# AntoineBlanot/LC2IS

Measured on AMD Instinct MI355X. Metric: training-step images/sec (512x512, ADE20K-150), higher is better.
Workload: dtype bf16; 1 GPU; BaseModelWithText ViT-B/16 + CLIP-text + decoder + fused head/CE train step, 512x512, 151 classes, text len 16, sgd; batch_per_gpu=32, global_batch=32, parallelism=dp1

## Files before the change

include/lc2is_hip.h:

```cpp
#ifndef LC2IS_HIP_H
#define LC2IS_HIP_H
#include <stddef.h>
#include <stdint.h>

#ifdef __cplusplus
extern "C" {
#endif

#define LC2IS_ACT_NONE 0
#define LC2IS_ACT_QUICK_GELU 1
#define LC2IS_ACT_RELU 2
#define LC2IS_ACT_DQUICK_GELU 3
#define LC2IS_ACT_DRELU 4
#define LC2IS_ACT_QUICK_GELU_GRAD 5
#define LC2IS_ACT_MUL_AUX 6
#define LC2IS_ACT_GELU_ERF 7
#define LC2IS_ACT_DGELU_ERF 8
#define LC2IS_ACT_ADD_AUX 9

#define LC2IS_INTERP_BICUBIC 0
#define LC2IS_INTERP_BILINEAR 1

typedef void* lc2is_stream_t;

// ... 103 lines not shown
int lc2is_transpose_bf16_batched(const void* src, int ld_src, long stride_src, void* dst, int ld_dst, long stride_dst,
                                 int R, int C, int batch, lc2is_stream_t stream);

int lc2is_patchify(const float* pixels, void* out_bf16, int ld_out, int B, int H, int W, int patch,
                   lc2is_stream_t stream);
int lc2is_vit_embed_fwd(const float* patch, int ld_patch, const float* cls, const float* pos, float* x,
                        int ldx, int B, int P, int C, lc2is_stream_t stream);
int lc2is_vit_embed_bwd(const float* dx, int ldx, float* dpos, float* dcls, void* dpatch_bf16, int ld_dpatch,
                        int B, int P, int C, int accumulate, lc2is_stream_t stream);
int lc2is_text_embed_fwd(const int64_t* ids, const float* tok, const float* pos, float* x, int ldx, int B,
                         int L, int C, int vocab, lc2is_stream_t stream);
int lc2is_text_embed_bwd(const int64_t* ids, const float* dx, int ldx, float* dtok, float* dpos, int B, int L,
                         int C, int vocab, int accumulate, lc2is_stream_t stream);
int lc2is_rows_copy_f32(const float* src, int S_src, int src_off, float* dst_f32, void* dst_bf16, int S_dst,
                        int dst_off, int B, int n, int C, lc2is_stream_t stream);
int lc2is_rows_copy_bf16(const void* src, int S_src, int src_off, float* dst_f32, void* dst_bf16, int S_dst,
                         int dst_off, int B, int n, int C, lc2is_stream_t stream);

int lc2is_sgd_step(float* params, const float* grads, float* momentum_buf, size_t n, float lr, float momentum,
                   float weight_decay, float grad_scale, lc2is_stream_t stream);
int lc2is_adamw_step(float* params, const float* grads, float* exp_avg, float* exp_avg_sq, size_t n, float lr,
                     float beta1, float beta2, float eps, float weight_decay, int step, float grad_scale,
                     lc2is_stream_t stream);

size_t lc2is_head_upsample_ce_workspace_bytes(int B, int h, int w, int C, int S, int mode, int want_grad);
int lc2is_head_upsample_ce(const float* scores_lo, int ld, const int64_t* labels, float* dscores_lo,
                           float* scores_hi, float* loss_sum, int B, int h, int w, int C, int S, int mode,
                           long ignore_index, float grad_scale, void* workspace, size_t workspace_bytes,
                           lc2is_stream_t stream);
int lc2is_head_upsample_ce_opts(const float* scores_lo, int ld, const int64_t* labels, float* dscores_lo,
                                float* scores_hi, float* loss_sum, int B, int h, int w, int C, int S, int mode,
                                long ignore_index, float grad_scale, const float* class_weight, float label_smoothing,
                                void* workspace, size_t workspace_bytes, lc2is_stream_t stream);
int lc2is_upsample_bwd_nchw(const float* dhi, float* dlo, int ld, int B, int h, int w, int C, int S, int mode,
                            lc2is_stream_t stream);
int lc2is_ce_nchw_fwd(const float* logits, const int64_t* labels, float* lse, float* loss_sum, int B, int C,
                      long HW, long ignore_index, lc2is_stream_t stream);
int lc2is_ce_nchw_bwd(const float* logits, const int64_t* labels, const float* lse, const float* grad_scale_dev,
                      float grad_scale, float* dlogits, int B, int C, long HW, long ignore_index,
                      lc2is_stream_t stream);
int lc2is_ce_nchw_fwd_opts(const float* logits, const int64_t* labels, float* lse, float* loss_sum, float* loss_px,
                           int B, int C, long HW, long ignore_index, const float* class_weight, float label_smoothing,
                           lc2is_stream_t stream);
int lc2is_ce_nchw_bwd_opts(const float* logits, const int64_t* labels, const float* lse, const float* grad_scale_dev,
                           float grad_scale, const float* grad_px, float* dlogits, int B, int C, long HW,
                           long ignore_index, const float* class_weight, float label_smoothing,
// ... 199 lines not shown
```

lc2is_amd/csrc/misc.hip:

```cpp
#include "common.h"
#include "lc2is_hip.h"

namespace {

__global__ __launch_bounds__(256) void shadow_refresh_kernel(const lc2is_shadow_desc* __restrict__ descs,
                                                              int ndesc) {
  __shared__ bf16_t tile[64][66];
  int lo = 0, hi = ndesc - 1;
  const int bid = blockIdx.x;
  while (lo < hi) {
    const int mid = (lo + hi + 1) >> 1;
    if (descs[mid].tile_start <= bid) lo = mid; else hi = mid - 1;
  }
  const lc2is_shadow_desc d = descs[lo];
  const int t = bid - d.tile_start;
  const int tk = (d.K + 63) / 64;
  const int n0 = (t / tk) * 64, k0 = (t % tk) * 64;
  const float* src = (const float*)d.src;
  bf16_t* dst = (bf16_t*)d.dst;
  bf16_t* dstT = (bf16_t*)d.dstT;
  const int tx = threadIdx.x & 15, ty = threadIdx.x >> 4;
#pragma unroll
  for (int r = 0; r < 4; ++r) {
    const int n = n0 + ty + 16 * r, k = k0 + 4 * tx;
// ... 220 lines not shown
    if (dst_b) *reinterpret_cast<uint2*>(dst_b + o) = make_uint2(pack_bf16x2(v.x, v.y), pack_bf16x2(v.z, v.w));
  }
}

__global__ __launch_bounds__(256) void sgd_kernel(float* p, const float* __restrict__ g, float* mom, size_t n4,
                                                   float lr, float momentum, float wd, float gscale) {
  for (size_t i = (size_t)blockIdx.x * 256 + threadIdx.x; i < n4; i += (size_t)gridDim.x * 256) {
    float4 pv = reinterpret_cast<float4*>(p)[i];
    const float4 gv = reinterpret_cast<const float4*>(g)[i];
    float d[4] = {gv.x * gscale + wd * pv.x, gv.y * gscale + wd * pv.y, gv.z * gscale + wd * pv.z,
                  gv.w * gscale + wd * pv.w};
    if (mom) {
      float4 mv = reinterpret_cast<float4*>(mom)[i];
      mv.x = momentum * mv.x + d[0]; mv.y = momentum * mv.y + d[1];
      mv.z = momentum * mv.z + d[2]; mv.w = momentum * mv.w + d[3];
      reinterpret_cast<float4*>(mom)[i] = mv;
      d[0] = mv.x; d[1] = mv.y; d[2] = mv.z; d[3] = mv.w;
    }
    pv.x -= lr * d[0]; pv.y -= lr * d[1]; pv.z -= lr * d[2]; pv.w -= lr * d[3];
    reinterpret_cast<float4*>(p)[i] = pv;
  }
}

__global__ __launch_bounds__(256) void adamw_kernel(float* p, const float* __restrict__ g, float* m, float* v,
                                                     size_t n4, float lr, float b1, float b2, float eps,
                                                     float wd, float bc1, float bc2, float gscale) {
  for (size_t i = (size_t)blockIdx.x * 256 + threadIdx.x; i < n4; i += (size_t)gridDim.x * 256) {
    float4 pv = reinterpret_cast<float4*>(p)[i];
    const float4 gv = reinterpret_cast<const float4*>(g)[i];
    float4 mv = reinterpret_cast<float4*>(m)[i], vv = reinterpret_cast<float4*>(v)[i];
    float* pp = &pv.x; const float* gp = &gv.x; float* mp = &mv.x; float* vp = &vv.x;
#pragma unroll
    for (int k = 0; k < 4; ++k) {
      const float gg = gp[k] * gscale;
      pp[k] *= (1.f - lr * wd);
      mp[k] = b1 * mp[k] + (1.f - b1) * gg;
      vp[k] = b2 * vp[k] + (1.f - b2) * gg * gg;
      const float denom = sqrtf(vp[k]) / sqrtf(bc2) + eps;
      pp[k] -= (lr / bc1) * (mp[k] / denom);
    }
    reinterpret_cast<float4*>(p)[i] = pv;
    reinterpret_cast<float4*>(m)[i] = mv;
    reinterpret_cast<float4*>(v)[i] = vv;
  }
}

// ... 124 lines not shown

extern "C" int lc2is_rows_copy_bf16(const void* src, int S_src, int src_off, float* dst_f32, void* dst_bf16,
                                    int S_dst, int dst_off, int B, int n, int C, lc2is_stream_t stream_) {
  hipStream_t stream = (hipStream_t)stream_;
  if (!src || (!dst_f32 && !dst_bf16)) return LC2IS_ERR_NULL;
  if (B <= 0 || n <= 0 || C <= 0 || C % 4 || src_off < 0 || dst_off < 0 || src_off + n > S_src ||
      dst_off + n > S_dst)
    return LC2IS_ERR_SHAPE;
  hipLaunchKernelGGL(rows_copy_bf16_kernel, dim3(ew_grid((size_t)B * n * C / 4)), dim3(256), 0, stream, (const bf16_t*)src,
                     S_src, src_off, dst_f32, (bf16_t*)dst_bf16, S_dst, dst_off, B, n, C);
  return lc2is_check_launch();
}

extern "C" int lc2is_sgd_step(float* params, const float* grads, float* momentum_buf, size_t n, float lr,
                              float momentum, float weight_decay, float grad_scale, lc2is_stream_t stream_) {
  hipStream_t stream = (hipStream_t)stream_;
  if (!params || !grads) return LC2IS_ERR_NULL;
  if (n == 0 || n % 4) return LC2IS_ERR_SHAPE;
  hipLaunchKernelGGL(sgd_kernel, dim3(ew_grid(n / 4)), dim3(256), 0, stream, params, grads, momentum_buf, n / 4,
                     lr, momentum, weight_decay, grad_scale);
  return lc2is_check_launch();
}

extern "C" int lc2is_adamw_step(float* params, const float* grads, float* exp_avg, float* exp_avg_sq, size_t n,
                                float lr, float beta1, float beta2, float eps, float weight_decay, int step,
                                float grad_scale, lc2is_stream_t stream_) {
  hipStream_t stream = (hipStream_t)stream_;
  if (!params || !grads || !exp_avg || !exp_avg_sq) return LC2IS_ERR_NULL;
  if (n == 0 || n % 4 || step < 1) return LC2IS_ERR_SHAPE;
  const float bc1 = 1.f - powf(beta1, (float)step), bc2 = 1.f - powf(beta2, (float)step);
  hipLaunchKernelGGL(adamw_kernel, dim3(ew_grid(n / 4)), dim3(256), 0, stream, params, grads, exp_avg,
                     exp_avg_sq, n / 4, lr, beta1, beta2, eps, weight_decay, bc1, bc2, grad_scale);
  return lc2is_check_launch();
}
```

lc2is_amd/nn/base.py:

```python
from __future__ import annotations

import torch
from torch import nn

from .. import ops


import os as _os

_WGRAD_SIDE = _os.environ.get("LC2IS_WGRAD_STREAM", "0") == "1"
_wgrad_streams: dict = {}


def wgrad_stream(device) -> torch.cuda.Stream:
    s = _wgrad_streams.get(device)
    if s is None:
        s = _wgrad_streams[device] = torch.cuda.Stream(device)
    return s


class _on_wgrad_stream:

    def __init__(self, *tensors):
        self.tensors = [t for t in tensors if t is not None]
# ... 86 lines not shown

def drop_branch_grad16(ds: DropSites | None, site: str, g32: torch.Tensor, g16: torch.Tensor | None) -> torch.Tensor:
    if ds is None:
        return g16 if g16 is not None else ops.cast_bf16(g32)
    return ops.dropout_rows_f32(g32, ds.p, ds.seeds[site], out_f32=None, out_bf16=True)[1]


def require_cuda(t: torch.Tensor, what: str) -> None:
    if not t.is_cuda:
        raise RuntimeError(
            f"lc2is_amd: {what} is on {t.device}; the MI355X path has no CPU fallback — move the module and its "
            "inputs to a HIP device (the CPU oracle lives in oracle/ and is test-only)")


class HipModule(nn.Module):

    def __init__(self) -> None:
        super().__init__()
        self._sh = None
        self._sh_table = None
        self._sh_versions = None
        self._sh_device = None
        self._sh_ptrs = []
        self._grad_ready_cb = None
        self._part_ready_cb = None

    def _build_shadows(self, device):
        raise NotImplementedError

    def _params_for_version(self):
        return list(self.parameters(recurse=True))

    def _ensure_ready(self):
        ps = self._params_for_version()
        dev = ps[0].device
        require_cuda(ps[0], f"{type(self).__name__} parameters")
        if self._sh is None or self._sh_device != dev or any(p.data_ptr() != q for p, q in zip(ps, self._sh_ptrs)):
            ns, entries = self._build_shadows(dev)
            self._sh = ns
            self._sh_table = ops.ShadowTable(entries, dev) if entries else None
            self._sh_device = dev
            self._sh_ptrs = [p.data_ptr() for p in ps]
            self._sh_versions = None
        vers = [p._version for p in ps]
        if vers != self._sh_versions:
            if self._sh_table is not None:
                self._sh_table.refresh()
            self._post_refresh()
            self._sh_versions = vers
        return self._sh

    def _post_refresh(self):
        pass

    def _grads_ready(self):
        if self._sh_device is not None:
            join_wgrad_stream(self._sh_device)
        if self._grad_ready_cb is not None:
            self._grad_ready_cb(self)

    def _part_grads_ready(self, part: nn.Module):
        if self._part_ready_cb is not None:
            if self._sh_device is not None:
                join_wgrad_stream(self._sh_device)
            self._part_ready_cb(self, part)

    def invalidate_shadows(self):
        self._sh_versions = None

    def _apply(self, fn, *args, **kwargs):
        self._sh = None
        return super()._apply(fn, *args, **kwargs)


def grad_buf(p: torch.Tensor):
    if p.grad is None:
        g = getattr(p, "_lc2is_grad", None)
        if g is None or g.shape != p.shape or g.device != p.device:
            g = torch.empty_like(p)
        p.grad = g
        return g, False
    return p.grad, True


class WgradBatch:

    _active = None

    def __init__(self, enabled: bool = True):
        self.enabled = enabled and _os.environ.get("LC2IS_WGRAD_GROUPED", "1") != "0"
        self.items = []
# ... 53 lines not shown
    return grad_buf(p)


GROUP_SKIP = 255


def granule_group_map(offsets, sizes, group_ids, dead=(), align: int = 64, ngroups: int | None = None) -> torch.Tensor:
    if not (len(offsets) == len(sizes) == len(group_ids)) or not len(offsets):
        raise ValueError("granule_group_map: offsets, sizes and group_ids must be non-empty and of one length")
    top = GROUP_SKIP if ngroups is None else int(ngroups)
    if not 1 <= top <= GROUP_SKIP:
        raise ValueError(f"granule_group_map: ngroups must be 1..{GROUP_SKIP}, got {ngroups}")
    dead = set(dead)
    ids, counts, at = [], [], 0
    for k, (o, n, g) in enumerate(zip(offsets, sizes, group_ids)):
        if o != at or o % align or n < 1:
            raise ValueError(f"granule_group_map: parameter {k} at offset {o} (size {n}) does not continue an aligned layout at {at}")
        if not 0 <= int(g) < top:
            raise ValueError(f"granule_group_map: parameter {k} has group id {g}; ids are 0..{top - 1}")
        ids.append(GROUP_SKIP if k in dead else int(g))
        counts.append((n + align - 1) // align)
        at = o + counts[-1] * align
    return torch.repeat_interleave(torch.tensor(ids, dtype=torch.uint8), torch.tensor(counts, dtype=torch.int64))


class ParamArena:

    ALIGN = 64

    def __init__(self, module: nn.Module):
        params = []
        seen = set()
        for p in module.parameters():
            if id(p) not in seen:
                seen.add(id(p))
                params.append(p)
        if not params:
            raise RuntimeError("ParamArena: module has no parameters")
        dev = params[0].device
        require_cuda(params[0], "ParamArena parameters")
        offs, total = [], 0
        for p in params:
            offs.append(total)
            total += (p.numel() + self.ALIGN - 1) // self.ALIGN * self.ALIGN
        self.flat = torch.zeros(total, dtype=torch.float32, device=dev)
        self.grad = torch.zeros(total, dtype=torch.float32, device=dev)
# ... 71 lines not shown
```

lc2is_amd/ops.py:

```python
from __future__ import annotations

import ctypes as C
import math
import os

import torch

from . import _lib

ACT_NONE, ACT_QUICK_GELU, ACT_RELU, ACT_DQUICK_GELU, ACT_DRELU, ACT_QUICK_GELU_GRAD, ACT_MUL_AUX = 0, 1, 2, 3, 4, 5, 6
ACT_GELU_ERF, ACT_DGELU_ERF, ACT_ADD_AUX = 7, 8, 9

_P, _I, _F, _Z, _L, _U64 = C.c_void_p, C.c_int, C.c_float, C.c_size_t, C.c_long, C.c_ulonglong
_ARGTYPES = {
    "lc2is_gemm_nt_bf16": [_P, _I, _P, _I, _P, _P, _I, _P, _I, _P, _I, _P, _I, _P, _I, _I, _I, _I, _I, _I, _P],
    "lc2is_gemm_nt_ln_xchg_bytes": [_I, _I],
    "lc2is_gemm_nt_ln_bf16": [_P, _I, _P, _I, _P, _P, _I, _P, _I, _P, _P, _F, _P, _I, _P, _P, _P, _Z, _I, _I, _I, _P],
    "lc2is_gemm_nt_bf16_batched": [_P, _I, _L, _P, _I, _L, _P, _I, _L, _P, _I, _L, _I, _I, _I, _I, _P],
    "lc2is_transpose_bf16_batched": [_P, _I, _L, _P, _I, _L, _I, _I, _I, _P],
    "lc2is_gemm_tn_workspace_bytes": [_I, _I, _I],
    "lc2is_gemm_tn_bf16": [_P, _I, _P, _I, _P, _I, _P, _I, _I, _I, _I, _P, _Z, _P],
    "lc2is_colsum_workspace_bytes": [_I, _I],
    "lc2is_colsum_bf16": [_P, _I, _P, _I, _I, _I, _P, _Z, _P],
    "lc2is_layernorm_fwd": [_P, _I, _I, _P, _P, _P, _I, _P, _I, _P, _P, _I, _I, _F, _P],
# ... 5 lines not shown
    "lc2is_attention_fwd": [_P, _I, _P, _I, _P, _I, _P, _I, _P, _P, _I, _I, _I, _I, _I, _F, _I, _P],
    "lc2is_attention_bwd": [_P, _I, _P, _I, _P, _I, _P, _I, _P, _I, _P, _I, _P, _I, _P, _I, _P, _P, _P,
                            _I, _I, _I, _I, _I, _F, _I, _P],
    "lc2is_attention_fwd_dropout": [_P, _I, _P, _I, _P, _I, _P, _I, _P, _P, _I, _I, _I, _I, _I, _F, _I, _F, _U64, _P],
    "lc2is_attention_bwd_dropout": [_P, _I, _P, _I, _P, _I, _P, _I, _P, _I, _P, _I, _P, _I, _P, _I, _P, _P, _P,
                                    _I, _I, _I, _I, _I, _F, _I, _F, _U64, _P],
    "lc2is_dropout_rows_f32": [_P, _I, _P, _I, _P, _I, _P, _I, _I, _I, _I, _F, _U64, _P],
    "lc2is_dropout_rows_bf16": [_P, _I, _P, _I, _I, _I, _F, _U64, _P],
    "lc2is_dropout_mask": [_P, _L, _I, _F, _U64, _P],
    "lc2is_shadow_refresh": [_P, _I, _I, _P],
    "lc2is_set_cu_budget": [_I],
    "lc2is_get_cu_budget": [],
    "lc2is_cast_f32_bf16": [_P, _I, _P, _I, _I, _I, _P],
    "lc2is_transpose_bf16": [_P, _I, _P, _I, _I, _I, _P],
    "lc2is_patchify": [_P, _P, _I, _I, _I, _I, _I, _P],
    "lc2is_vit_embed_fwd": [_P, _I, _P, _P, _P, _I, _I, _I, _I, _P],
    "lc2is_vit_embed_bwd": [_P, _I, _P, _P, _P, _I, _I, _I, _I, _I, _P],
    "lc2is_text_embed_fwd": [_P, _P, _P, _P, _I, _I, _I, _I, _I, _P],
    "lc2is_text_embed_bwd": [_P, _P, _I, _P, _P, _I, _I, _I, _I, _I, _P],
    "lc2is_rows_copy_bf16": [_P, _I, _I, _P, _P, _I, _I, _I, _I, _I, _P],
    "lc2is_rows_copy_f32": [_P, _I, _I, _P, _P, _I, _I, _I, _I, _I, _P],
    "lc2is_sgd_step": [_P, _P, _P, _Z, _F, _F, _F, _F, _P],
    "lc2is_adamw_step": [_P, _P, _P, _P, _Z, _F, _F, _F, _F, _F, _I, _F, _P],
    "lc2is_grad_sumsq_blocks": [_Z],
    "lc2is_grad_sumsq_workspace_bytes": [_Z],
    "lc2is_grad_sumsq": [_P, _Z, _P, _Z, _P],
    "lc2is_optim_ctrl_update": [_P, _P, _P, _I, _P, _I, _F, _F, _I, _F, _F, _P],
    "lc2is_sgd_step_ctrl": [_P, _P, _P, _Z, _P, _F, _F, _I, _P],
    "lc2is_adamw_step_ctrl": [_P, _P, _P, _P, _Z, _P, _F, _F, _F, _F, _I, _P],
    "lc2is_sgd_step_groups": [_P, _P, _P, _Z, _P, _P, _P, _I, _F, _I, _P],
    "lc2is_adamw_step_groups": [_P, _P, _P, _P, _Z, _P, _P, _P, _I, _F, _F, _F, _I, _P],
    "lc2is_ema_update_ctrl": [_P, _P, _Z, _P, _F, _I, _I, _I, _P],
    "lc2is_swap_f32": [_P, _P, _Z, _P],
    "lc2is_head_upsample_ce_workspace_bytes": [_I, _I, _I, _I, _I, _I, _I],
    "lc2is_head_upsample_ce": [_P, _I, _P, _P, _P, _P, _I, _I, _I, _I, _I, _I, C.c_long, _F, _P, _Z, _P],
    "lc2is_ce_nchw_fwd": [_P, _P, _P, _P, _I, _I, C.c_long, C.c_long, _P],
    "lc2is_ce_nchw_bwd": [_P, _P, _P, _P, _F, _P, _I, _I, C.c_long, C.c_long, _P],
    "lc2is_head_upsample_ce_opts": [_P, _I, _P, _P, _P, _P, _I, _I, _I, _I, _I, _I, C.c_long, _F, _P, _F, _P, _Z, _P],
    "lc2is_ce_nchw_fwd_opts": [_P, _P, _P, _P, _P, _I, _I, C.c_long, C.c_long, _P, _F, _P],
    "lc2is_ce_nchw_fwd_workspace_bytes": [_I, C.c_long],
    "lc2is_ce_nchw_fwd_ordered": [_P, _P, _P, _P, _P, _I, _I, C.c_long, C.c_long, _P, _F, _P, _Z, _P],
    "lc2is_ce_nchw_bwd_opts": [_P, _P, _P, _P, _F, _P, _P, _I, _I, C.c_long, C.c_long, _P, _F, _P],
    "lc2is_upsample_bwd_nchw": [_P, _P, _I, _I, _I, _I, _I, _I, _I, _P],
    "lc2is_head_upsample_px": [_P, _I, _P, _P, _I, _I, _I, _I, _I, _I, _L, _P],
    "lc2is_ohem_select_workspace_bytes": [_L],
    "lc2is_ohem_select": [_P, _P, _P, _L, _I, _L, _F, _L, _P, _P, _Z, _P],
# ... 470 lines not shown
        self._keep = []
        for i, (src, dst, dstT) in enumerate(entries):
            if src.dim() == 1:
                src = src.unsqueeze(0)
                dst = dst.unsqueeze(0) if dst is not None and dst.dim() == 1 else dst
            f32copy = dst is not None and dst.dtype == torch.float32
            _chk(src, torch.float32, "shadow src")
            _chk(dst, torch.float32 if f32copy else torch.bfloat16, "shadow dst")
            _chk(dstT, torch.bfloat16, "shadow dstT")
            if f32copy and dstT is not None:
                raise RuntimeError("lc2is_amd: fp32 shadow copies have no transposed twin")
            if not src.is_contiguous():
                raise RuntimeError("lc2is_amd: shadow source must be contiguous")
            N, K = src.shape
            if K % 4 or (dstT is not None and N % 4):
                raise RuntimeError(f"lc2is_amd: shadow shape [{N},{K}] not supported")
            if dst is not None and tuple(dst.shape) != (N, K):
                raise RuntimeError("lc2is_amd: shadow dst shape mismatch")
            if dstT is not None and tuple(dstT.shape) != (K, N):
                raise RuntimeError("lc2is_amd: shadow dstT shape mismatch")
            descs[i] = ShadowDesc(src.data_ptr(), _ptr(dst), _ptr(dstT), N, K, _ld(dst), _ld(dstT), start, int(f32copy))
            start += ((N + 63) // 64) * ((K + 63) // 64)
            self._keep.append((src, dst, dstT))
        self.n = len(entries)
        self.total_tiles = start
        raw = bytes(descs)
        self.dev = torch.frombuffer(bytearray(raw), dtype=torch.uint8).to(device)

    def refresh(self):
        rc = _fn("lc2is_shadow_refresh")(self.dev.data_ptr(), self.n, self.total_tiles, _stream())
        _lib.check(rc, "shadow_refresh")


def cast_bf16(src: torch.Tensor, out: torch.Tensor | None = None):
    _chk(src, torch.float32, "src")
    M, Cc = src.shape
    out = out if out is not None else torch.empty((M, Cc), dtype=torch.bfloat16, device=src.device)
    _chk(out, torch.bfloat16, "out")
    _lib.check(_fn("lc2is_cast_f32_bf16")(_ptr(src), _ld(src), _ptr(out), _ld(out), M, Cc, _stream()), "cast")
    return out


def transpose_bf16(src: torch.Tensor, out: torch.Tensor | None = None):
    _chk(src, torch.bfloat16, "src")
    R, Cc = src.shape
    out = out if out is not None else torch.empty((Cc, R), dtype=torch.bfloat16, device=src.device)
    _chk(out, torch.bfloat16, "out")
    _lib.check(_fn("lc2is_transpose_bf16")(_ptr(src), _ld(src), _ptr(out), _ld(out), R, Cc, _stream()),
               "transpose")
    return out
# ... 48 lines not shown
    V, Cc = dtok.shape
    _lib.check(_fn("lc2is_text_embed_bwd")(_ptr(ids), _ptr(dx), _ld(dx), _ptr(dtok), _ptr(dpos), B, L, Cc, V,
                                           int(accumulate), _stream()), "text_embed_bwd")


def rows_copy(src, S_src: int, src_off: int, S_dst: int, dst_off: int, B: int, n: int, *, dst_f32=None,
              dst_bf16=None):
    sb = src.dtype == torch.bfloat16
    _chk(src, torch.bfloat16 if sb else torch.float32, "src")
    Cc = src.shape[1]
    if not src.is_contiguous() or src.shape[0] != B * S_src:
        raise RuntimeError("lc2is_amd.rows_copy: src must be contiguous [B*S_src, C]")
    for t in (dst_f32, dst_bf16):
        if t is not None and (not t.is_contiguous() or tuple(t.shape) != (B * S_dst, Cc)):
            raise RuntimeError("lc2is_amd.rows_copy: dst must be contiguous [B*S_dst, C]")
    _lib.check(_fn("lc2is_rows_copy_bf16" if sb else "lc2is_rows_copy_f32")(_ptr(src), S_src, src_off, _ptr(dst_f32), _ptr(dst_bf16),
                                                                            S_dst, dst_off, B, n, Cc, _stream()), "rows_copy")


def sgd_step(params, grads, momentum_buf, lr, momentum=0.0, weight_decay=0.0, grad_scale=1.0):
    _chk(params, torch.float32, "params", 1); _chk(grads, torch.float32, "grads", 1)
    _lib.check(_fn("lc2is_sgd_step")(_ptr(params), _ptr(grads), _ptr(momentum_buf), params.numel(), lr, momentum,
                                     weight_decay, grad_scale, _stream()), "sgd_step")


def adamw_step(params, grads, m, v, lr, beta1, beta2, eps, weight_decay, step, grad_scale=1.0):
    _chk(params, torch.float32, "params", 1); _chk(grads, torch.float32, "grads", 1)
    _lib.check(_fn("lc2is_adamw_step")(_ptr(params), _ptr(grads), _ptr(m), _ptr(v), params.numel(), lr, beta1,
                                       beta2, eps, weight_decay, int(step), grad_scale, _stream()), "adamw_step")


OPTIM_CTRL_WORDS = 12
(CTRL_CALLS, CTRL_APPLIED, CTRL_SKIPPED, CTRL_FINITE, CTRL_GRAD_NORM, CTRL_CLIP_COEF, CTRL_LR, CTRL_BC1, CTRL_BC2, CTRL_GRAD_MUL,
 CTRL_APPLY) = range(11)


def _chk_ctrl(ctrl):
    _chk(ctrl, torch.int32, "ctrl", 1)
    if ctrl.numel() != OPTIM_CTRL_WORDS:
        raise RuntimeError(f"lc2is_amd: ctrl must be an int32 [{OPTIM_CTRL_WORDS}] control block (lc2is_optim_ctrl)")


def _chk_same_numel(name, params, *others):
    for t in others:
        if t is not None:
            _chk(t, torch.float32, name + " buffer", 1)
# ... 920 lines not shown
```

lc2is_amd/step.py:

```python
from __future__ import annotations

import contextlib
import math
import os
import re

import torch
from torch import nn

from . import ops
from .nn.base import HipModule, ParamArena


_DEFAULT_LR = 1e-5


def _accepts_ohem(model) -> bool:
    import inspect
    fl = getattr(model, "forward_loss", None)
    return fl is not None and "ohem" in inspect.signature(fl).parameters


def _accepts_dice(model) -> bool:
    import inspect
    fl = getattr(model, "forward_loss", None)
    return fl is not None and "dice" in inspect.signature(fl).parameters


def lr_table_from_torch(make_scheduler, base_lr: float, steps: int) -> torch.Tensor:
    if steps < 1:
        raise ValueError("lr_table_from_torch: steps must be >= 1")
    opt = torch.optim.SGD([torch.nn.Parameter(torch.zeros(1))], lr=base_lr)
    sched = make_scheduler(opt)
    rates = []
# ... 188 lines not shown
            depth[m.group(1)] = max(depth.get(m.group(1), 0), int(m.group(2)) + 1)
    merged = {}
    for name, prm in named:
        wd = float(weight_decay)
        if no_decay and (prm.dim() == 1 or name.endswith(("position_embedding.weight", "token_embedding.weight"))
                         or any(sub in name for sub in extra)):
            wd = 0.0
        scale, best = 1.0, -1
        for prefix, f in lr_scales.items():
            if name.startswith(prefix) and len(prefix) > best:
                scale, best = float(f), len(prefix)
        if layer_decay is not None:
            m = _TOWER_LAYER.match(name)
            if m:
                scale *= float(layer_decay) ** (depth[m.group(1)] - int(m.group(2)))
            else:
                for tower, L in depth.items():
                    if name.startswith((tower + ".embeddings.", tower + ".pre_layrnorm.")):
                        scale *= float(layer_decay) ** (L + 1)
        merged.setdefault((scale, wd), []).append(name)
    return [dict(params=names, lr_scale=scale, weight_decay=wd) for (scale, wd), names in merged.items()]


class TrainStep:

    def __init__(self, model: nn.Module, *, optimizer: str = "sgd", lr: float = _DEFAULT_LR, momentum: float = 0.0,
                 weight_decay: float = 0.0, betas=(0.9, 0.999), eps: float = 1e-8, reducer=None,
                 ignore_index: int | None = None, criterion: nn.Module | None = None, lr_schedule=None,
                 schedule_steps: int | None = None, max_grad_norm: float | None = None, skip_nonfinite: bool = False,
                 device_state: bool = False, param_groups=None, ema_decay: float | None = None, ema_warmup: bool = False,
                 ema_every: int = 1) -> None:
        _check_ema_args(ema_decay, ema_warmup, ema_every)
        device_path = bool(device_state or skip_nonfinite or lr_schedule is not None or max_grad_norm is not None
                           or param_groups is not None or ema_decay is not None)
        groups = None
        if param_groups is not None:
            groups, group_of = _resolve_param_groups(model, param_groups, weight_decay)
        if max_grad_norm is not None and not float(max_grad_norm) > 0.0:
            raise ValueError(f"TrainStep: max_grad_norm must be > 0 (or None / inf for no clipping), got {max_grad_norm}")
        table = _lr_table(lr_schedule, schedule_steps, lr) if (device_path or schedule_steps is not None) else None
        self._loss_opts = False
        self._ohem = False
        self._dice = False
        if criterion is not None:
            from .nn.loss import AuxiliaryLoss, CrossEntropyLoss, DiceCrossEntropyLoss, OhemCrossEntropyLoss
            if not isinstance(criterion, (CrossEntropyLoss, nn.CrossEntropyLoss)) or isinstance(criterion, AuxiliaryLoss):
# ... 8 lines not shown
            self._ohem = isinstance(criterion, OhemCrossEntropyLoss)
            if self._ohem and not _accepts_ohem(model):
                raise TypeError("TrainStep: an OhemCrossEntropyLoss needs a model whose forward_loss takes ohem= "
                                "(BaseModelWithText); the compose models do not select hard pixels")
            self._dice = isinstance(criterion, DiceCrossEntropyLoss)
            if self._dice and not _accepts_dice(model):
                raise TypeError("TrainStep: a DiceCrossEntropyLoss needs a model whose forward_loss takes dice= "
                                "(BaseModelWithText); the compose models have no Dice head")
        self.criterion = criterion
        self.model = model
        self.arena = ParamArena(model)
        self.kind = optimizer.lower()
        if self.kind not in ("sgd", "adamw"):
            raise ValueError("TrainStep: optimizer must be 'sgd' or 'adamw'")
        self.lr, self.momentum, self.weight_decay, self.betas, self.eps = lr, momentum, weight_decay, betas, eps
        dev = self.arena.flat.device
        self.mom = torch.zeros_like(self.arena.flat) if (self.kind == "sgd" and momentum != 0.0) else None
        if self.kind == "adamw":
            self.m, self.v = torch.zeros_like(self.arena.flat), torch.zeros_like(self.arena.flat)
        self.t = 0
        self.reducer = reducer
        self.ignore_index = -100 if ignore_index is None else ignore_index
        self._hip_modules = [m for m in model.modules() if isinstance(m, HipModule)]
        if reducer is not None:
            reducer.attach(model, self.arena)
        self._dev = dev
        self._ctrl = None
        if device_path:
            self._ctrl = torch.zeros(ops.OPTIM_CTRL_WORDS, dtype=torch.int32, device=dev)
            self._ctrl_f = self._ctrl.view(torch.float32)
            self.lr_table = table.to(dev)
            self.max_grad_norm = float("inf") if max_grad_norm is None else float(max_grad_norm)
            self.skip_nonfinite = bool(skip_nonfinite)
            self.reverse_walk = False
        self._groups = groups
        if groups is not None:
            self.arena.set_groups([group_of[id(p)] for p in self.arena.params], len(groups))
            self._group_table = torch.tensor([[g["lr_scale"], g["weight_decay"]] for g in groups], dtype=torch.float32).to(dev)
        self.ema, self._ema_swapped = None, False
        self.ema_decay = None if ema_decay is None else float(ema_decay)
        self.ema_warmup, self.ema_every = bool(ema_warmup), int(ema_every)
        if ema_decay is not None:
            self._ema_w = 1.0 - self.ema_decay
            self.ema_reverse_walk = True
            self.ema = self.arena.flat.clone()

# ... 122 lines not shown
        sd = {"format": 1, "meta": self._state_meta(), "t": int(self.t)}
        for k, b in self._state_buffers().items():
            sd[k] = b.detach().to("cpu", copy=True)
        if self._ctrl is not None:
            sd["lr_table"] = self.lr_table.detach().to("cpu", copy=True)
        if self._groups is not None:
            sd["group_table"] = self._group_table.detach().to("cpu", copy=True)
        return sd

    def load_state_dict(self, sd: dict) -> None:
        if self._ema_swapped:
            raise RuntimeError("TrainStep.load_state_dict: not inside ema_weights()")
        if not isinstance(sd, dict) or "meta" not in sd or "t" not in sd:
            raise ValueError("TrainStep.load_state_dict: not a TrainStep.state_dict()")
        check_train_state(sd["meta"], self._state_meta())
        bufs = self._state_buffers()
        for k, b in bufs.items():
            src = sd.get(k)
            if not isinstance(src, torch.Tensor) or src.dtype != b.dtype or src.shape != b.shape:
                raise ValueError(f"TrainStep.load_state_dict: '{k}' must be a {b.dtype} tensor of shape {tuple(b.shape)}")
        for k, b in bufs.items():
            b.copy_(sd[k])
        self.t = int(sd["t"])

    def step(self, inputs: dict, labels: torch.Tensor) -> torch.Tensor:
        if self._ema_swapped:
            raise RuntimeError("TrainStep.step: inside ema_weights() the parameters are the EMA; leave the block before training")
        arena = self.arena
        arena.zero_grad(set_to_none=True)
        if self.reducer is not None:
            self.reducer.begin_step()
        if self._ohem:
            c = self.criterion
            loss = self.model.forward_loss(inputs, labels, self.ignore_index, weight=c.weight,
                                           label_smoothing=float(c.label_smoothing), reduction=c.reduction,
                                           ohem=c.ohem if c.training else None)
            if c.training:
                c.last_labels, c.last_info = self.model.last_ohem
        elif self._dice:
            c = self.criterion
            loss = self.model.forward_loss(inputs, labels, self.ignore_index, dice=c.dice)
            c.last_stats = self.model.last_dice
        elif self._loss_opts:
            c = self.criterion
            loss = self.model.forward_loss(inputs, labels, self.ignore_index, weight=c.weight,
                                           label_smoothing=float(c.label_smoothing), reduction=c.reduction)
        else:
            loss = self.model.forward_loss(inputs, labels, self.ignore_index)
        loss.backward()
        live = arena.finalize_grads()
        gscale = 1.0
        if self.reducer is not None:
            self.reducer.finish_step()
            gscale = 1.0 / self.reducer.world_size
        self.t += 1
        segs = [(0, arena.numel)] if (self.weight_decay == 0.0 or live == [(0, arena.numel)]) else live
        if self._ctrl is not None:
            ctrl = self._ctrl
            b1, b2 = self.betas if self.kind == "adamw" else (0.0, 0.0)
            partials, flags = ops.grad_sumsq(arena.grad)
            ops.optim_ctrl_update(ctrl, partials, flags, self.lr_table, grad_scale=gscale, max_norm=self.max_grad_norm,
                                  skip_nonfinite=self.skip_nonfinite, beta1=b1, beta2=b2)
            if self._groups is not None:
                gmap = arena.group_map()
                if self.kind == "sgd":
                    ops.sgd_step_groups(arena.flat, arena.grad, self.mom, ctrl, gmap, self._group_table, self.momentum,
                                        reverse=self.reverse_walk)
                else:
                    ops.adamw_step_groups(arena.flat, arena.grad, self.m, self.v, ctrl, gmap, self._group_table, self.betas[0],
                                          self.betas[1], self.eps, reverse=self.reverse_walk)
                segs = []
            for lo, hi in segs:
                sl = slice(lo, hi)
                if self.kind == "sgd":
                    ops.sgd_step_ctrl(arena.flat[sl], arena.grad[sl], None if self.mom is None else self.mom[sl], ctrl,
                                      self.momentum, self.weight_decay, reverse=self.reverse_walk)
                else:
                    ops.adamw_step_ctrl(arena.flat[sl], arena.grad[sl], self.m[sl], self.v[sl], ctrl, self.betas[0],
                                        self.betas[1], self.eps, self.weight_decay, reverse=self.reverse_walk)
# ... 19 lines not shown
        if self._ema_swapped:
            raise RuntimeError("TrainStep.capture: inside ema_weights() the parameters are the EMA; leave the block before training")
        if self.kind == "adamw" and self._ctrl is None:
            raise RuntimeError("TrainStep.capture: AdamW bias correction is step-dependent; capture supports SGD")
        if hasattr(self.model, "overlap_text") and os.environ.get("LC2IS_GRAPH_OVERLAP", "1") == "0":
            self.model.overlap_text = False
        from .nn.base import DropoutRng
        DropoutRng.last.clear()
        static_in = {k: v.clone() for k, v in inputs.items()}
        static_lb = labels.clone()
        side = torch.cuda.Stream()
        side.wait_stream(torch.cuda.current_stream())
        with torch.cuda.stream(side):
            for _ in range(warmup):
                self.step(static_in, static_lb)
        torch.cuda.current_stream().wait_stream(side)
        torch.cuda.synchronize()
        if DropoutRng.last:
            raise RuntimeError("TrainStep.capture: the model has active dropout / drop-path sites "
                               f"({len(DropoutRng.last)}); their per-step seeds cannot be captured — train eagerly or set the rates to 0")
        prev = getattr(self, "_captured", None)
        if prev is not None:
            prev.release()
        graph = torch.cuda.CUDAGraph()
        t_before = self.t
        mark0 = ops.captured_tables_mark()
        with torch.cuda.graph(graph, stream=side):
            static_loss = self.step(static_in, static_lb)
        mark1 = ops.captured_tables_mark()
        self.t = t_before

        def replay(new_inputs: dict, new_labels: torch.Tensor) -> torch.Tensor:
            if self._ema_swapped:
                raise RuntimeError("TrainStep replay: inside ema_weights() the parameters are the EMA; leave the block before "
                                   "training")
            for k, v in new_inputs.items():
                if v is not static_in[k]:
                    static_in[k].copy_(v, non_blocking=True)
            if new_labels is not static_lb:
                static_lb.copy_(new_labels, non_blocking=True)
            graph.replay()
            self.t += 1
            return static_loss

        state = {"live": True}

        def release() -> None:
            if not state["live"]:
                return
            state["live"] = False
            torch.cuda.synchronize()
            graph.reset()
            ops.release_captured_tables_range(mark0, mark1)
            if getattr(self, "_captured", None) is replay:
                self._captured = None

        replay.static_inputs, replay.static_labels, replay.graph, replay.release = static_in, static_lb, graph, release
        self._captured = replay
        return replay
```

Before: 1031 images/s.

## Fuse SGD update with bf16 shadow weight refresh in one kernel

Adds an SGD kernel that walks the shadow-table tiles, updates fp32 params and momentum in place, and writes the bf16 (and transposed) shadow copies in the same pass. A segment kernel updates the remaining parameters that have no shadows. Modules are then marked as having current shadows, so the separate refresh pass on the next forward is skipped. This removes one full read of the weights and several launches per step, at the cost of extra version-guard bookkeeping and a new path that only applies to eager SGD without groups, EMA or graph capture.

```diff
diff --git a/include/lc2is_hip.h b/include/lc2is_hip.h
--- a/include/lc2is_hip.h
+++ b/include/lc2is_hip.h
@@ -149,6 +149,14 @@
 int lc2is_adamw_step(float* params, const float* grads, float* exp_avg, float* exp_avg_sq, size_t n, float lr,
                      float beta1, float beta2, float eps, float weight_decay, int step, float grad_scale,
                      lc2is_stream_t stream);
+
+#define LC2IS_MAX_SGD_SEGMENTS 64
+int lc2is_sgd_step_shadow(const lc2is_shadow_desc* descs, int ndesc, int total_tiles, float* params, const float* grads,
+                          float* momentum_buf, size_t n, float lr, float momentum, float weight_decay, float grad_scale,
+                          lc2is_stream_t stream);
+int lc2is_sgd_step_segments(float* params, const float* grads, float* momentum_buf, size_t n, const size_t* seg_lo,
+                            const size_t* seg_hi, int nseg, float lr, float momentum, float weight_decay, float grad_scale,
+                            lc2is_stream_t stream);
 
 size_t lc2is_head_upsample_ce_workspace_bytes(int B, int h, int w, int C, int S, int mode, int want_grad);
 int lc2is_head_upsample_ce(const float* scores_lo, int ld, const int64_t* labels, float* dscores_lo,
diff --git a/lc2is_amd/csrc/misc.hip b/lc2is_amd/csrc/misc.hip
--- a/lc2is_amd/csrc/misc.hip
+++ b/lc2is_amd/csrc/misc.hip
@@ -266,6 +266,105 @@
   }
 }
 
+__device__ __forceinline__ void sgd_update4(float4& pv, const float4 gv, float4& mv, const bool has_mom, const float lr,
+                                            const float momentum, const float wd, const float gscale) {
+  float d[4] = {gv.x * gscale + wd * pv.x, gv.y * gscale + wd * pv.y, gv.z * gscale + wd * pv.z,
+                gv.w * gscale + wd * pv.w};
+  if (has_mom) {
+    mv.x = momentum * mv.x + d[0]; mv.y = momentum * mv.y + d[1];
+    mv.z = momentum * mv.z + d[2]; mv.w = momentum * mv.w + d[3];
+    d[0] = mv.x; d[1] = mv.y; d[2] = mv.z; d[3] = mv.w;
+  }
+  pv.x -= lr * d[0]; pv.y -= lr * d[1]; pv.z -= lr * d[2]; pv.w -= lr * d[3];
+}
+
+__global__ __launch_bounds__(256) void sgd_shadow_kernel(const lc2is_shadow_desc* __restrict__ descs, int ndesc,
+                                                          const float* arena_lo, const float* arena_hi, ptrdiff_t goff,
+                                                          ptrdiff_t moff, int has_mom, float lr, float momentum, float wd,
+                                                          float gscale) {
+  __shared__ bf16_t tile[64][66];
+  int lo = 0, hi = ndesc - 1;
+  const int bid = blockIdx.x;
+  while (lo < hi) {
+    const int mid = (lo + hi + 1) >> 1;
+    if (descs[mid].tile_start <= bid) lo = mid; else hi = mid - 1;
+  }
+  const lc2is_shadow_desc d = descs[lo];
+  const int t = bid - d.tile_start;
+  const int tk = (d.K + 63) / 64;
+  const int n0 = (t / tk) * 64, k0 = (t % tk) * 64;
+  float* src = (float*)d.src;
+  if (src < arena_lo || src + (size_t)d.N * d.K > arena_hi) return;
+  bf16_t* dst = (bf16_t*)d.dst;
+  bf16_t* dstT = (bf16_t*)d.dstT;
+  const int tx = threadIdx.x & 15, ty = threadIdx.x >> 4;
+#pragma unroll
+  for (int r = 0; r < 4; ++r) {
+    const int n = n0 + ty + 16 * r, k = k0 + 4 * tx;
+    float4 v = make_float4(0.f, 0.f, 0.f, 0.f);
+    if (n < d.N && k < d.K) {
+      float* pp = src + (size_t)n * d.K + k;
+      v = *reinterpret_cast<const float4*>(pp);
+      const float4 gv = *reinterpret_cast<const float4*>(pp + goff);
+      float4 mv = make_float4(0.f, 0.f, 0.f, 0.f);
+      if (has_mom) mv = *reinterpret_cast<const float4*>(pp + moff);
+      sgd_update4(v, gv, mv, has_mom != 0, lr, momentum, wd, gscale);
+      if (has_mom) *reinterpret_cast<float4*>(pp + moff) = mv;
+      *reinterpret_cast<float4*>(pp) = v;
+    }
+    const bf16_t b0 = f32_to_bf16(v.x), b1 = f32_to_bf16(v.y), b2 = f32_to_bf16(v.z), b3 = f32_to_bf16(v.w);
+    if (d.flags & 1) {
+      if (dst && n < d.N && k < d.K) *reinterpret_cast<float4*>((float*)d.dst + (size_t)n * d.ld_dst + k) = v;
+    } else if (dst && n < d.N && k < d.K) {
+      uint2 pk = make_uint2((unsigned)b0 | ((unsigned)b1 << 16), (unsigned)b2 | ((unsigned)b3 << 16));
+      *reinterpret_cast<uint2*>(dst + (size_t)n * d.ld_dst + k) = pk;
+    }
+    tile[ty + 16 * r][4 * tx + 0] = b0;
+    tile[ty + 16 * r][4 * tx + 1] = b1;
+    tile[ty + 16 * r][4 * tx + 2] = b2;
+    tile[ty + 16 * r][4 * tx + 3] = b3;
+  }
+  if (!dstT) return;
+  __syncthreads();
+#pragma unroll
+  for (int r = 0; r < 4; ++r) {
+    const int k = k0 + ty + 16 * r, n = n0 + 4 * tx;
+    if (k < d.K && n < d.N) {
+      const int kk = ty + 16 * r;
+      uint2 pk = make_uint2((unsigned)tile[4 * tx][kk] | ((unsigned)tile[4 * tx + 1][kk] << 16),
+                            (unsigned)tile[4 * tx + 2][kk] | ((unsigned)tile[4 * tx + 3][kk] << 16));
+      *reinterpret_cast<uint2*>(dstT + (size_t)k * d.ld_dstT + n) = pk;
+    }
+  }
+}
+
+struct sgd_segs {
+  unsigned lo4[LC2IS_MAX_SGD_SEGMENTS];
+  unsigned pre4[LC2IS_MAX_SGD_SEGMENTS + 1];
+};
+
+__global__ __launch_bounds__(256) void sgd_segments_kernel(float* p, const float* __restrict__ g, float* mom,
+                                                            const sgd_segs segs, int nseg, float lr, float momentum, float wd,
+                                                            float gscale) {
+  __shared__ unsigned s_lo[LC2IS_MAX_SGD_SEGMENTS], s_pre[LC2IS_MAX_SGD_SEGMENTS + 1];
+  if ((int)threadIdx.x < nseg) s_lo[threadIdx.x] = segs.lo4[threadIdx.x];
+  if ((int)threadIdx.x <= nseg) s_pre[threadIdx.x] = segs.pre4[threadIdx.x];
+  __syncthreads();
+  const size_t total = s_pre[nseg];
+  int s = 0;
+  for (size_t j = (size_t)blockIdx.x * 256 + threadIdx.x; j < total; j += (size_t)gridDim.x * 256) {
+    while (j >= s_pre[s + 1]) ++s;
+    const size_t i = (size_t)s_lo[s] + (j - s_pre[s]);
+    float4 pv = reinterpret_cast<float4*>(p)[i];
+    const float4 gv = reinterpret_cast<const float4*>(g)[i];
+    float4 mv = make_float4(0.f, 0.f, 0.f, 0.f);
+    if (mom) mv = reinterpret_cast<float4*>(mom)[i];
+    sgd_update4(pv, gv, mv, mom != nullptr, lr, momentum, wd, gscale);
+    if (mom) reinterpret_cast<float4*>(mom)[i] = mv;
+    reinterpret_cast<float4*>(p)[i] = pv;
+  }
+}
+
 __global__ __launch_bounds__(256) void adamw_kernel(float* p, const float* __restrict__ g, float* m, float* v,
                                                      size_t n4, float lr, float b1, float b2, float eps,
                                                      float wd, float bc1, float bc2, float gscale) {
@@ -436,6 +535,45 @@
   return lc2is_check_launch();
 }
 
+extern "C" int lc2is_sgd_step_shadow(const lc2is_shadow_desc* descs_dev, int ndesc, int total_tiles, float* params,
+                                     const float* grads, float* momentum_buf, size_t n, float lr, float momentum,
+                                     float weight_decay, float grad_scale, lc2is_stream_t stream_) {
+  hipStream_t stream = (hipStream_t)stream_;
+  if (!descs_dev || !params || !grads) return LC2IS_ERR_NULL;
+  if (ndesc <= 0 || total_tiles <= 0 || n == 0 || n % 4 || ((uintptr_t)params & 15u) || ((uintptr_t)grads & 15u) ||
+      ((uintptr_t)momentum_buf & 15u))
+    return LC2IS_ERR_SHAPE;
+  const ptrdiff_t goff = grads - params, moff = momentum_buf ? momentum_buf - params : 0;
+  hipLaunchKernelGGL(sgd_shadow_kernel, dim3(total_tiles), dim3(256), 0, stream, descs_dev, ndesc, (const float*)params,
+                     (const float*)(params + n), goff, moff, momentum_buf ? 1 : 0, lr, momentum, weight_decay, grad_scale);
+  return lc2is_check_launch();
+}
+
+extern "C" int lc2is_sgd_step_segments(float* params, const float* grads, float* momentum_buf, size_t n,
+                                       const size_t* seg_lo, const size_t* seg_hi, int nseg, float lr, float momentum,
+                                       float weight_decay, float grad_scale, lc2is_stream_t stream_) {
+  hipStream_t stream = (hipStream_t)stream_;
+  if (!params || !grads || (nseg > 0 && (!seg_lo || !seg_hi))) return LC2IS_ERR_NULL;
+  if (nseg < 0 || nseg > LC2IS_MAX_SGD_SEGMENTS || n == 0 || n % 4 || (n >> 34) || ((uintptr_t)params & 15u) ||
+      ((uintptr_t)grads & 15u) || ((uintptr_t)momentum_buf & 15u))
+    return LC2IS_ERR_SHAPE;
+  sgd_segs segs = {};
+  size_t total4 = 0, prev_hi = 0;
+  for (int s = 0; s < nseg; ++s) {
+    const size_t lo = seg_lo[s], hi = seg_hi[s];
+    if (lo >= hi || hi > n || lo % 64 || hi % 64 || lo < prev_hi) return LC2IS_ERR_SHAPE;
+    segs.lo4[s] = (unsigned)(lo / 4);
+    segs.pre4[s] = (unsigned)total4;
+    total4 += (hi - lo) / 4;
+    prev_hi = hi;
+  }
+  segs.pre4[nseg] = (unsigned)total4;
+  if (nseg == 0) return 0;
+  hipLaunchKernelGGL(sgd_segments_kernel, dim3(ew_grid(total4)), dim3(256), 0, stream, params, grads, momentum_buf, segs,
+                     nseg, lr, momentum, weight_decay, grad_scale);
+  return lc2is_check_launch();
+}
+
 extern "C" int lc2is_adamw_step(float* params, const float* grads, float* exp_avg, float* exp_avg_sq, size_t n,
                                 float lr, float beta1, float beta2, float eps, float weight_decay, int step,
                                 float grad_scale, lc2is_stream_t stream_) {
diff --git a/lc2is_amd/nn/base.py b/lc2is_amd/nn/base.py
--- a/lc2is_amd/nn/base.py
+++ b/lc2is_amd/nn/base.py
@@ -1,4 +1,6 @@
 from __future__ import annotations
+
+import bisect
 
 import torch
 from torch import nn
@@ -132,6 +134,7 @@
         self._sh_versions = None
         self._sh_device = None
         self._sh_ptrs = []
+        self._sh_guard = None
         self._grad_ready_cb = None
         self._part_ready_cb = None
 
@@ -153,11 +156,14 @@
             self._sh_ptrs = [p.data_ptr() for p in ps]
             self._sh_versions = None
         vers = [p._version for p in ps]
+        if self._sh_guard is not None and self._sh_guard[0]._version != self._sh_guard[1]:
+            self._sh_versions = None
         if vers != self._sh_versions:
             if self._sh_table is not None:
                 self._sh_table.refresh()
             self._post_refresh()
             self._sh_versions = vers
+            self._sh_guard = None
         return self._sh
 
     def _post_refresh(self):
@@ -177,6 +183,17 @@
 
     def invalidate_shadows(self):
         self._sh_versions = None
+        self._sh_guard = None
+
+    def mark_shadows_current(self, flat: torch.Tensor | None = None):
+        self._sh_versions = [p._version for p in self._params_for_version()]
+        self._sh_guard = None if flat is None else (flat, flat._version)
+
+    def shadows_match_params(self) -> bool:
+        if self._sh is None or self._sh_table is None:
+            return False
+        ps = self._params_for_version()
+        return len(ps) == len(self._sh_ptrs) and all(p.data_ptr() == q for p, q in zip(ps, self._sh_ptrs))
 
     def _apply(self, fn, *args, **kwargs):
         self._sh = None
@@ -276,6 +293,41 @@
         counts.append((n + align - 1) // align)
         at = o + counts[-1] * align
     return torch.repeat_interleave(torch.tensor(ids, dtype=torch.uint8), torch.tensor(counts, dtype=torch.int64))
+
+
+def step_tail_segments(offsets, sizes, covered, align: int = 64):
+    if len(offsets) != len(sizes) or not len(offsets):
+        raise ValueError("step_tail_segments: offsets and sizes must be non-empty and of one length")
+    at = 0
+    for k, (o, n) in enumerate(zip(offsets, sizes)):
+        if o != at or o % align or n < 1:
+            raise ValueError(f"step_tail_segments: parameter {k} at offset {o} (size {n}) does not continue an aligned layout at {at}")
+        at = o + (n + align - 1) // align * align
+    total, offs = at, list(offsets)
+    got = [0] * len(offsets)
+    end = -1
+    for lo, n in sorted((int(lo), int(n)) for lo, n in covered):
+        if n < 1 or lo < 0 or lo + n > total:
+            raise ValueError(f"step_tail_segments: a covered range [{lo}, {lo + n}) lies outside the arena of {total} elements")
+        if lo < end:
+            raise ValueError(f"step_tail_segments: the element at {lo} is covered twice")
+        end = lo + n
+        k = bisect.bisect_right(offs, lo) - 1
+        if lo + n > offsets[k] + sizes[k]:
+            raise ValueError(f"step_tail_segments: a covered range [{lo}, {lo + n}) does not lie inside one parameter")
+        got[k] += n
+    segs = []
+    for k, (o, n) in enumerate(zip(offsets, sizes)):
+        if got[k] == n:
+            continue
+        if got[k]:
+            raise ValueError(f"step_tail_segments: parameter {k} is covered in part ({got[k]} of {n} elements)")
+        hi = o + (n + align - 1) // align * align
+        if segs and segs[-1][1] == o:
+            segs[-1] = (segs[-1][0], hi)
+        else:
+            segs.append((o, hi))
+    return segs
 
 
 class ParamArena:
diff --git a/lc2is_amd/ops.py b/lc2is_amd/ops.py
--- a/lc2is_amd/ops.py
+++ b/lc2is_amd/ops.py
@@ -51,6 +51,8 @@
     "lc2is_rows_copy_f32": [_P, _I, _I, _P, _P, _I, _I, _I, _I, _I, _P],
     "lc2is_sgd_step": [_P, _P, _P, _Z, _F, _F, _F, _F, _P],
     "lc2is_adamw_step": [_P, _P, _P, _P, _Z, _F, _F, _F, _F, _F, _I, _F, _P],
+    "lc2is_sgd_step_shadow": [_P, _I, _I, _P, _P, _P, _Z, _F, _F, _F, _F, _P],
+    "lc2is_sgd_step_segments": [_P, _P, _P, _Z, _P, _P, _I, _F, _F, _F, _F, _P],
     "lc2is_grad_sumsq_blocks": [_Z],
     "lc2is_grad_sumsq_workspace_bytes": [_Z],
     "lc2is_grad_sumsq": [_P, _Z, _P, _Z, _P],
@@ -567,10 +569,27 @@
             descs[i] = ShadowDesc(src.data_ptr(), _ptr(dst), _ptr(dstT), N, K, _ld(dst), _ld(dstT), start, int(f32copy))
             start += ((N + 63) // 64) * ((K + 63) // 64)
             self._keep.append((src, dst, dstT))
-        self.n = len(entries)
-        self.total_tiles = start
-        raw = bytes(descs)
-        self.dev = torch.frombuffer(bytearray(raw), dtype=torch.uint8).to(device)
+        self._set(descs, start, device)
+
+    def _set(self, descs, total_tiles, device):
+        self.n, self.total_tiles, self.host = len(descs), total_tiles, descs
+        self.sources = [(src.data_ptr(), src.numel()) for src, _, _ in self._keep]
+        self.dev = torch.frombuffer(bytearray(bytes(descs)), dtype=torch.uint8).to(device)
+
+    @classmethod
+    def merged(cls, tables, device):
+        self = cls.__new__(cls)
+        descs = (ShadowDesc * sum(t.n for t in tables))()
+        self._keep = []
+        i = start = 0
+        for t in tables:
+            for d in t.host:
+                descs[i] = ShadowDesc(d.src, d.dst, d.dstT, d.N, d.K, d.ld_dst, d.ld_dstT, start + d.tile_start, d.flags)
+                i += 1
+            start += t.total_tiles
+            self._keep += t._keep
+        self._set(descs, start, device)
+        return self
 
     def refresh(self):
         rc = _fn("lc2is_shadow_refresh")(self.dev.data_ptr(), self.n, self.total_tiles, _stream())
@@ -665,6 +684,37 @@
     _chk(params, torch.float32, "params", 1); _chk(grads, torch.float32, "grads", 1)
     _lib.check(_fn("lc2is_sgd_step")(_ptr(params), _ptr(grads), _ptr(momentum_buf), params.numel(), lr, momentum,
                                      weight_decay, grad_scale, _stream()), "sgd_step")
+
+
+MAX_SGD_SEGMENTS = 64
+
+
+def sgd_step_shadow(table, params, grads, momentum_buf, lr, momentum=0.0, weight_decay=0.0, grad_scale=1.0):
+    _chk(params, torch.float32, "params", 1); _chk(grads, torch.float32, "grads", 1)
+    _chk_same_numel("sgd_step_shadow", params, grads, momentum_buf)
+    lo, hi = params.data_ptr(), params.data_ptr() + 4 * params.numel()
+    if getattr(table, "_inside", None) != (lo, hi):
+        if any(ptr < lo or ptr + 4 * n > hi for ptr, n in table.sources):
+            raise RuntimeError("lc2is_amd.sgd_step_shadow: the table has a source outside params")
+        table._inside = (lo, hi)
+    _lib.check(_fn("lc2is_sgd_step_shadow")(table.dev.data_ptr(), table.n, table.total_tiles, _ptr(params), _ptr(grads),
+                                            _ptr(momentum_buf), params.numel(), lr, momentum, weight_decay, grad_scale,
+                                            _stream()), "sgd_step_shadow")
+
+
+def split_segments(segments, limit: int = MAX_SGD_SEGMENTS):
+    segments = [(int(lo), int(hi)) for lo, hi in segments]
+    return [segments[i:i + limit] for i in range(0, len(segments), limit)]
+
+
+def sgd_step_segments(params, grads, momentum_buf, segments, lr, momentum=0.0, weight_decay=0.0, grad_scale=1.0):
+    _chk(params, torch.float32, "params", 1); _chk(grads, torch.float32, "grads", 1)
+    _chk_same_numel("sgd_step_segments", params, grads, momentum_buf)
+    for run in split_segments(segments):
+        lo = (C.c_size_t * len(run))(*[s[0] for s in run])
+        hi = (C.c_size_t * len(run))(*[s[1] for s in run])
+        _lib.check(_fn("lc2is_sgd_step_segments")(_ptr(params), _ptr(grads), _ptr(momentum_buf), params.numel(), lo, hi, len(run),
+                                                  lr, momentum, weight_decay, grad_scale, _stream()), "sgd_step_segments")
 
 
 def adamw_step(params, grads, m, v, lr, beta1, beta2, eps, weight_decay, step, grad_scale=1.0):
diff --git a/lc2is_amd/step.py b/lc2is_amd/step.py
--- a/lc2is_amd/step.py
+++ b/lc2is_amd/step.py
@@ -9,7 +9,7 @@
 from torch import nn
 
 from . import ops
-from .nn.base import HipModule, ParamArena
+from .nn.base import HipModule, ParamArena, step_tail_segments
 
 
 _DEFAULT_LR = 1e-5
@@ -244,6 +244,20 @@
     return [dict(params=names, lr_scale=scale, weight_decay=wd) for (scale, wd), names in merged.items()]
 
 
+def step_tail_enabled(env=None) -> bool:
+    v = (os.environ if env is None else env).get("LC2IS_STEP_TAIL", "1")
+    if v not in ("0", "1"):
+        raise ValueError(f"LC2IS_STEP_TAIL must be 0 or 1, got {v!r}")
+    return v == "1"
+
+
+def step_tail_eligible(*, kind: str, device_path: bool, groups: bool, ema: bool, weight_decay: float, all_live: bool,
+                       capturing: bool, enabled: bool = True) -> bool:
+    if not enabled or kind != "sgd" or device_path or groups or ema or capturing:
+        return False
+    return weight_decay == 0.0 or all_live
+
+
 class TrainStep:
 
     def __init__(self, model: nn.Module, *, optimizer: str = "sgd", lr: float = _DEFAULT_LR, momentum: float = 0.0,
@@ -298,6 +312,8 @@
         self.reducer = reducer
         self.ignore_index = -100 if ignore_index is None else ignore_index
         self._hip_modules = [m for m in model.modules() if isinstance(m, HipModule)]
+        self._tail_enabled = step_tail_enabled()
+        self._tail_sig, self._tail = None, None
         if reducer is not None:
             reducer.attach(model, self.arena)
         self._dev = dev
@@ -466,6 +482,28 @@
         for k, b in bufs.items():
             b.copy_(sd[k])
         self.t = int(sd["t"])
+
+    def _tail_plan(self):
+        arena = self.arena
+        base = arena.flat.data_ptr()
+        sig = (base,) + tuple(id(m._sh_table) for m in self._hip_modules)
+        if sig == self._tail_sig:
+            return self._tail
+        self._tail_sig, self._tail = sig, None
+        ready = [m for m in self._hip_modules if m.shadows_match_params()]
+        if any(type(m)._post_refresh is not HipModule._post_refresh for m in ready):
+            return None
+        covered = [(ptr - base, n) for m in ready for ptr, n in m._sh_table.sources]
+        if any(off % 4 for off, _ in covered):
+            return None
+        covered = [(off // 4, n) for off, n in covered]
+        try:
+            segs = step_tail_segments(arena.offsets, [p.numel() for p in arena.params], covered)
+        except ValueError:
+            return None
+        table = ops.ShadowTable.merged([m._sh_table for m in ready], arena.flat.device) if ready else None
+        self._tail = dict(ready=ready, table=table, segs=segs)
+        return self._tail
 
     def step(self, inputs: dict, labels: torch.Tensor) -> torch.Tensor:
         if self._ema_swapped:
@@ -499,6 +537,23 @@
             gscale = 1.0 / self.reducer.world_size
         self.t += 1
         segs = [(0, arena.numel)] if (self.weight_decay == 0.0 or live == [(0, arena.numel)]) else live
+        plan = None
+        if step_tail_eligible(kind=self.kind, device_path=self._ctrl is not None, groups=self._groups is not None,
+                              ema=self.ema is not None, weight_decay=self.weight_decay, all_live=live == [(0, arena.numel)],
+                              capturing=torch.cuda.is_current_stream_capturing(), enabled=self._tail_enabled):
+            plan = self._tail_plan()
+        if plan is not None:
+            if plan["table"] is not None:
+                ops.sgd_step_shadow(plan["table"], arena.flat, arena.grad, self.mom, self.lr, self.momentum, self.weight_decay,
+                                    gscale)
+            ops.sgd_step_segments(arena.flat, arena.grad, self.mom, plan["segs"], self.lr, self.momentum, self.weight_decay,
+                                  gscale)
+            for m in self._hip_modules:
+                if m in plan["ready"]:
+                    m.mark_shadows_current(arena.flat)
+                else:
+                    m.invalidate_shadows()
+            return loss.detach()
         if self._ctrl is not None:
             ctrl = self._ctrl
             b1, b2 = self.betas if self.kind == "adamw" else (0.0, 0.0)
@@ -564,6 +619,8 @@
         prev = getattr(self, "_captured", None)
         if prev is not None:
             prev.release()
+        for m in self._hip_modules:
+            m.invalidate_shadows()
         graph = torch.cuda.CUDAGraph()
         t_before = self.t
         mark0 = ops.captured_tables_mark()
@@ -582,6 +639,8 @@
             if new_labels is not static_lb:
                 static_lb.copy_(new_labels, non_blocking=True)
             graph.replay()
+            for m in self._hip_modules:
+                m.invalidate_shadows()
             self.t += 1
             return static_loss
 
```

Result: no change. 1035 images/s (median of 6 runs) (+0.4%).
